# KushalChaudhari-16/Medical-Image-Denoising-Using-Diffusion

Measured on AMD Instinct MI355X. Metric: denoised images/sec, 256x256 x50 DDIM steps, higher is better.
Workload: dtype f32 (split-fp16 x3 MFMA, fp32 accumulate); 1 GPU; batch=8/GPU 256x256 grayscale, 50-iteration reverse loop (noise_steps=50, inference_steps=50), random-init 12.8M-param UNet (BASELINE.json configs[1]); batch_per_gpu=8, global_batch=8, parallelism=single, collective=none

## Files before the change

### medical-image-denoising-using-diffusion_amd/csrc/conv_mfma_f16x3.hip

```cpp
#include "f16x3_common.h"
#include <cstdlib>
#include <type_traits>
#ifdef MIDD_CONV_TIMING
#include <cstdio>
#include <cstring>
#include <string>
#include <vector>
#endif

namespace midd {

template <int KS, int STRIDE, int TW, int MT, int NT, int WM, int WN, int CBT = 0>
struct Conv16Geom {
    static constexpr int NW = WM * WN;
    static constexpr int NTHREADS = NW * 64;
    static constexpr int BM = WM * MT * 16;
    static constexpr int TH = BM / TW;
    static constexpr int IH = (TH - 1) * STRIDE + KS;
    static constexpr int IW = (TW - 1) * STRIDE + KS;
    static constexpr int NPIX = IH * IW;
    static constexpr int CB = CBT ? CBT : conv16_cb(KS);
    static constexpr bool WIDE = (KS == 3 && CB == 2);
    static constexpr int QPP = 4 * CB;
    static constexpr int NSLOT = NPIX * QPP;
// ... 67 lines not shown
    float* const stat_lds = reinterpret_cast<float*>(wring + RING * WSLICE);
    float* const add_lds = stat_lds + G::STAT_FLOATS;
    float* const gnp = add_lds + G::ADD_FLOATS;

    const int tid = threadIdx.x;
    const int lane = tid & 63;
    const int wave = __builtin_amdgcn_readfirstlane(tid >> 6);
    const int wn = wave % WN;
    const int wm = wave / WN;
    const int p16 = lane & 15;
    const int kq = lane >> 4;

    const int tiles_per_img = a.tiles_x * a.tiles_y;
    const int b = blockIdx.x / a.wgs_per_img;
    int trem = blockIdx.x - b * a.wgs_per_img;
    int oy0 = (trem / a.tiles_x) * TH, ox0 = (trem % a.tiles_x) * TW;

    const int Cin = a.C0 + a.C1;
    const int nblk = Cin >> 4;
    constexpr int CB = G::CB, QPP = G::QPP;
    const int nchunks = (nblk + CB - 1) / CB;
    const int ntiles_total = a.Cout >> 4;
    const int ntile_wg = blockIdx.y * (WN * NT);
    const int res_steps = RES ? a.res_steps : 0;
    const int total_steps = conv16_num_steps(Cin, TAPS, G::CB) + res_steps;

    const char* const wbase = reinterpret_cast<const char*>(a.wpack) + (size_t)ntile_wg * 2048;
    const size_t wstep_bytes = (size_t)ntiles_total * 2048;
    const int lane16 = lane * 16;
    int wr_step = 0, wr_slot = 0;
    const char* wr_src = wbase;
#ifdef MIDD_DMA_CHECK
    constexpr unsigned SENT_W = 0x7FFF7FFFu;
    constexpr unsigned SENT_A = 0x7FC0DEADu;
    unsigned dma_bad = 0;
    auto sent4 = [](unsigned v) { typedef unsigned u32x4_ __attribute__((ext_vector_type(4))); return __builtin_bit_cast(f32x4, (u32x4_){v, v, v, v}); };
    auto has_sent = [](const auto& q, unsigned v) {
        typedef unsigned u32x4_ __attribute__((ext_vector_type(4)));
        const u32x4_ u = __builtin_bit_cast(u32x4_, q);
        return (unsigned)((u[0] == v) | (u[1] == v) | (u[2] == v) | (u[3] == v));
    };
#endif
    auto issue_w = [&]() {
        char* slot = wring + wr_slot * WSLICE;
#ifdef MIDD_DMA_CHECK
#pragma unroll
        for (int i = 0; i < PPW; ++i) {
            int piece = (WM == 1) ? wave * PPW + i : wave + i * NW;
            if (piece >= G::WPIECES) piece -= G::WPIECES;
            lds_store_raw(slot + piece * 1024 + lane16, sent4(SENT_W));
        }
// ... 47 lines not shown
            const unsigned byte_off = (unsigned)max(g_off[s], 0) * 64u;
            dma16(base + byte_off, raw + (wave + s * NW) * 1024);
        }
    };
    float rscale = RAW_PRESCALE;
    auto transform = [&](int c) {
        const int blk = CB * c + sblk;
        if (blk >= nblk) return;
        const int ch = (blk << 4) + (q8 & 3) * 4;
        f32x4 rq[APW];
#pragma unroll
        for (int s = 0; s < APW; ++s) rq[s] = *reinterpret_cast<const f32x4*>(raw + (tid + s * NTHREADS) * 16);
#ifdef MIDD_DMA_CHECK
#pragma unroll
        for (int s = 0; s < APW; ++s) dma_bad |= has_sent(rq[s], SENT_A);
#endif
        f32x4 sc = {rscale, rscale, rscale, rscale}, sh = {0.f, 0.f, 0.f, 0.f};
        if (a.prologue != PRO_RAW) {
            sc = *reinterpret_cast<const f32x4*>(gnp + ch);
            sh = *reinterpret_cast<const f32x4*>(gnp + Cin + ch);
        }
        char* base = img + sblk * 2 * PLANE + (q8 & 3) * 8;
        typedef unsigned u32x2 __attribute__((ext_vector_type(2)));
        if (c == 0 && tile_pad) {
#pragma unroll
            for (int s = 0; s < APW; ++s) {
                const int slot = tid + s * NTHREADS;
                if (g_off[s] == -1) {
                    *reinterpret_cast<u32x2*>(base + (slot / QPP) * 32) = (u32x2){0u, 0u};
                    *reinterpret_cast<u32x2*>(base + PLANE + (slot / QPP) * 32) = (u32x2){0u, 0u};
                }
            }
        }
#pragma unroll
        for (int s = 0; s < APW; ++s) {
            const int slot = tid + s * NTHREADS;
            float v[4];
#pragma unroll
            for (int e = 0; e < 4; ++e) v[e] = __builtin_fmaf(rq[s][e], sc[e], sh[e]);
#if defined(C16_ABL) && C16_ABL == 4
            if (false) {
#else
            if (a.prologue == PRO_GN_SILU) {
#endif
#pragma unroll
                for (int e = 0; e < 4; ++e) {
                    const float d = __builtin_fmaf(__builtin_amdgcn_exp2f(v[e]), 1.0f / ACT_PRESCALE, 1.0f / ACT_PRESCALE);
// ... 12 lines not shown
    };

    int frag_base[MT];
#pragma unroll
    for (int mt = 0; mt < MT; ++mt) {
        const int pp = (wm * MT + mt) * 16 + p16;
        const int py = pp / TW, px = pp - py * TW;
        frag_base[mt] = ((py * STRIDE) * IW + px * STRIDE) * 32 + (kq & 1) * 16;
    }
    int frag_full[MT];
#pragma unroll
    for (int mt = 0; mt < MT; ++mt) frag_full[mt] = frag_base[mt] + (kq >> 1) * 2 * PLANE;
    const int wfrag_off = (wn * NT) * 2048 + lane * 16;

    f32x4 acc[MT][NT];
#pragma unroll
    for (int mt = 0; mt < MT; ++mt)
#pragma unroll
        for (int nt = 0; nt < NT; ++nt) acc[mt][nt] = (f32x4){0.f, 0.f, 0.f, 0.f};

    constexpr int D = RING - 1;
    const int ntile0 = ntile_wg + wn * NT;
    TS_DECL
    issue_a(0);
#pragma unroll
    for (int i = 0; i < D; ++i) issue_w();
#if !(defined(C16_ABL) && C16_ABL == 6)
    if (a.prologue == PRO_GN || a.prologue == PRO_GN_SILU)
        gn_prologue_lds(a.gn_tot0, a.C0, a.gn_bs0, a.gn_tot1, a.C1, a.gn_bs1, a.stat_rep, a.gn_gamma, a.gn_beta, a.gn_eps, a.gn_inv_n, b,
                        (a.prologue == PRO_GN_SILU) ? SILU_ARG_FACTOR : ACT_PRESCALE, gnp, tid, NTHREADS, a.status);
#endif
    stat_word* const raw_acc = reinterpret_cast<stat_word*>(gnp);
    if (a.prologue == PRO_RAW && a.gn_tot0 != nullptr && wave == 0)
        raw_sumsq_lds(a.gn_tot0, a.C0, a.gn_bs0, a.gn_tot1, a.C1, a.gn_bs1, a.stat_rep, b, raw_acc, lane);
    stat_word* const res_acc = reinterpret_cast<stat_word*>(gnp + 2 * Cin);
    if (res_steps > 0 && a.res_tot0 != nullptr && wave == NW - 1)
        raw_sumsq_lds(a.res_tot0, a.res_C0, a.res_bs0, a.res_tot1, a.res_C1, a.res_bs1, a.stat_rep, b, res_acc, lane);
    {
        const int trow = (a.temb != nullptr) ? a.trow[b] : 0;
        for (int i = tid; i < G::ADD_FLOATS; i += NTHREADS) {
            const int co = ntile_wg * 16 + i;
            add_lds[i] = a.bias[co] + (a.temb != nullptr ? a.temb[(size_t)trow * a.temb_stride + co] : 0.f);
        }
    }
    wait_vm_and_barrier<0>();
    float oscale = a.out_scale;
    if (a.prologue == PRO_RAW) {
        rscale = a.raw_scale_fixed;
        if (a.gn_tot0 != nullptr) {
            bool bad;
            const int ex = __builtin_amdgcn_readfirstlane(raw_prescale_exp(raw_acc, &bad));
            rscale = pow2f(ex);
            if (bad && tid == 0 && a.status != nullptr) atomicOr(a.status, (int)STATUS_NONFINITE);
        }
        oscale = a.out_scale / rscale;
    }
    float res_in = 1.0f, res_rescale = 1.0f;
    if (res_steps > 0) {
        if (a.res_tot0 != nullptr) {
            bool bad;
            res_in = pow2f(__builtin_amdgcn_readfirstlane(raw_prescale_exp(res_acc, &bad)));
            if (bad && tid == 0 && a.status != nullptr) atomicOr(a.status, (int)STATUS_NONFINITE);
        }
        res_rescale = a.out_scale * res_in / a.res_scale;
        oscale = a.res_scale / res_in;
    }
    transform(0);
    if constexpr (WM == 1) {
        asm volatile("s_waitcnt lgkmcnt(0)" ::: "memory");
        __builtin_amdgcn_s_barrier();
        asm volatile("" ::: "memory");
    }

    TS(TS_PROLOGUE)
    int rd_slot = 0;
    half8 xh[MT], xl[MT];
    auto load_x = [&](const int (&xo)[MT]) {
#pragma unroll
        for (int mt = 0; mt < MT; ++mt) {
            xh[mt] = *reinterpret_cast<const half8*>(img + xo[mt]);
            xl[mt] = *reinterpret_cast<const half8*>(img + xo[mt] + PLANE);
        }
    };
    auto mfma_step = [&]() {
        const char* wslot = wring + rd_slot * WSLICE + wfrag_off;
        rd_slot = (rd_slot + 1 == RING) ? 0 : rd_slot + 1;
        half8 wh[NT], wl[NT];
#pragma unroll
        for (int nt = 0; nt < NT; ++nt) {
            wh[nt] = *reinterpret_cast<const half8*>(wslot + nt * 2048);
// ... 229 lines not shown
                lds_store_raw(my_stat + NT * 16 + nt * 16, ssq[nt]);
            }
        }
        constexpr int ROWF = 2 * NT * 16;
        constexpr int NCOL = WN * NT * 16;
        auto fold = [&](int i) {
            const int which = i / NCOL, col = i - which * NCOL;
            const int wn_i = col / (NT * 16), c = col - wn_i * (NT * 16);
            float t = 0.f;
#pragma unroll
            for (int m = 0; m < WM; ++m) t += stat_lds[(m * WN + wn_i) * ROWF + which * (NT * 16) + c];
            return t;
        };
        static_assert(G::RAW_BYTES + G::IMG_BYTES + RING * WSLICE >= (NCOL + 2) * STAT_WORDS * 8, "block accumulators in the staging buffers (raw, image, ring: contiguous, idle here)");
        if constexpr (G::RAW_BYTES < (NCOL + 2) * STAT_WORDS * 8) {
            asm volatile("s_waitcnt lgkmcnt(0)" ::: "memory");
            __builtin_amdgcn_s_barrier();
            asm volatile("" ::: "memory");
        }
        stat_publish(a.stat_tot, b, a.Cout, a.stat_bs, a.stat_rep, (blockIdx.x - b * a.wgs_per_img) % a.stat_rep, ntile_wg * 16, NCOL,
                     fold, reinterpret_cast<stat_word*>(raw), tid, NTHREADS);
    };

    for (;;) {
        const int next_tile = trem + a.wgs_per_img;
        const bool has_next_tile = next_tile < tiles_per_img;
        for (int c = 0; c < nchunks; ++c) {
            const bool more_in_tile = (c + 1 < nchunks);
            const bool more = more_in_tile || has_next_tile;
            const int next_chunk = more_in_tile ? c + 1 : 0;
            const bool full = (CB == 2) && (2 * c + 1 < nblk);
            if (!more_in_tile && has_next_tile) set_tile(next_tile);
            auto run_chunk = [&](auto more_t) {
                constexpr bool MORE = decltype(more_t)::value;
                if (full) {
#pragma unroll
                    for (int tap = 0; tap < TAPS; ++tap) {
                        const int dy = tap / KS, dx = tap - dy * KS;
                        int xo[MT];
#pragma unroll
                        for (int mt = 0; mt < MT; ++mt) xo[mt] = frag_full[mt] + (dy * IW + dx) * 32;
                        if (MORE && tap >= 1 && tap <= D) k_step(std::true_type{}, false, false, next_chunk, xo);
                        else                              k_step(std::false_type{}, tap == 0, MORE && tap == 0, next_chunk, xo);
                    }
                } else {
#pragma unroll
                    for (int hs = 0; hs < HSTEPS; ++hs) {
                        const int t0 = 2 * hs, t1 = (2 * hs + 1 < TAPS) ? 2 * hs + 1 : 0;
                        const int o0 = ((t0 / KS) * IW + (t0 % KS)) * 32, o1 = ((t1 / KS) * IW + (t1 % KS)) * 32;
                        const int to = (kq >> 1) ? o1 : o0;
                        int xo[MT];
#pragma unroll
                        for (int mt = 0; mt < MT; ++mt) xo[mt] = frag_base[mt] + to;
// ... 18 lines not shown
#ifdef MIDD_CONV_TIMING
                    ts_after_epi = true;
#endif
                }
#if !(defined(C16_ABL) && C16_ABL == 5)
                transform(next_chunk);
#endif
                TS(TS_TRANSFORM)
                if constexpr (WM == 1) {
                    asm volatile("s_waitcnt lgkmcnt(0)" ::: "memory");
                    __builtin_amdgcn_s_barrier();
                    asm volatile("" ::: "memory");
                }
            } else {
                run_chunk(std::false_type{});
                res_phase();
                TS(TS_RES)
            }
        }
        if (!has_next_tile) break;
    }
    asm volatile("s_waitcnt vmcnt(0)" ::: "memory");
    TS(TS_CHUNK_WAIT)
    epilogue();
    TS(TS_EPILOGUE)
    publish_stats();
#ifdef MIDD_DMA_CHECK
    if (dma_bad && a.status != nullptr) atomicOr(a.status, (int)STATUS_DMA_EARLY);
#endif
    TS(TS_PUBLISH)
#ifdef MIDD_CONV_TIMING
    if (tid == 0) {
        ts_acc[TS_TOTAL] = ts_last - ts_t0;
        ts_acc[TS_REAL] = __builtin_amdgcn_s_memrealtime() - ts_r0;
        ts_acc[TS_WGS] = 1;
        for (int k = 0; k < TS_N; ++k) atomicAdd(&g_conv_timing[a.dbg_slot][k], ts_acc[k]);
    }
#endif
}

#ifdef MIDD_CONV_TIMING
static std::vector<std::string> g_timing_names;
static int conv_timing_slot(int ks, int st, int tw, int mt, int nt, int wm, int wn, int oh, int cin, int cout, int B, int ring, int wgs) {
    char buf[160];
    snprintf(buf, sizeof buf, "k%d s%d tile(%d,%d,%d,%d,%d) ring%d out%d^2 %d->%d B%d wgs%d", ks, st, tw, mt, nt, wm, wn, ring, oh, cin, cout, B, wgs);
    for (size_t i = 0; i < g_timing_names.size(); ++i) if (g_timing_names[i] == buf) return (int)i;
    if (g_timing_names.size() >= 63) return 63;
    g_timing_names.push_back(buf);
    return (int)g_timing_names.size() - 1;
// ... 3 lines not shown
    (void)hipDeviceSynchronize();
    (void)hipMemcpyFromSymbol(h, HIP_SYMBOL(g_conv_timing), sizeof h);
    static const char* names[] = {"barrier", "dma-issue", "frag+mfma", "chunk-wait", "transform", "epilogue", "prologue", "wait-after-epi", "dma-wait", "res-phase", "publish"};
    for (size_t i = 0; i < g_timing_names.size(); ++i) {
        const double tot = (double)h[i][TS_TOTAL], wgs = (double)h[i][TS_WGS];
        if (wgs == 0) continue;
        printf("%-70s cyc/wg %9.0f clk %.2f GHz |", g_timing_names[i].c_str(), tot / wgs, tot / (double)h[i][TS_REAL] * 0.1);
        for (int k = 0; k < 11; ++k) printf(" %s %4.1f%%", names[k], 100.0 * (double)h[i][k] / tot);
        printf("\n");
    }
    memset(h, 0, sizeof h);
    (void)hipMemcpyToSymbol(HIP_SYMBOL(g_conv_timing), h, sizeof h);
    fflush(stdout);
}
#endif
template <int KS, int STRIDE, int TW, int MT, int NT, int WM, int WN, bool RES, int CBT = 0>
static hipError_t launch16(const ConvArgs& a0, hipStream_t s) {
    using G = Conv16Geom<KS, STRIDE, TW, MT, NT, WM, WN, CBT>;
    ConvArgs a = a0;
    a.tiles_x = (a.OW + TW - 1) / TW;
    a.tiles_y = (a.OH + G::TH - 1) / G::TH;
    const int ny = a.Cout / (WN * NT * 16);
    a.wgs_per_img = conv16_wgs_per_img(a.tiles_x * a.tiles_y, a.B, ny, a.persist_wgs);
    dim3 grid(a.B * a.wgs_per_img, ny);
#ifdef MIDD_CONV_TIMING
    a.dbg_slot = conv_timing_slot(KS, STRIDE, TW, MT * 10 + G::CB, NT, WM, WN, a.OH, a.C0 + a.C1, a.Cout, a.B, G::RING, (int)grid.x * (int)grid.y);
#endif
    if constexpr (G::LDS_BYTES <= 160 * 1024 && (G::RING - 2) * G::PPW + G::APW <= 60) {
        const int lds_bytes = G::lds_bytes(a.C0 + a.C1);
        if (lds_bytes > 160 * 1024) return hipErrorInvalidValue;
        {
            static int raised[MIDD_MAX_DEVICES] = {};
            hipError_t e = ensure_dynamic_lds(reinterpret_cast<const void*>(&conv_mfma_f16x3_kernel<KS, STRIDE, TW, MT, NT, WM, WN, RES, CBT>), lds_bytes, raised);
            if (e != hipSuccess) return e;
        }
        if ((double)a.H * a.W * 64.0 >= 4294967296.0) return hipErrorInvalidValue;
        hipLaunchKernelGGL((conv_mfma_f16x3_kernel<KS, STRIDE, TW, MT, NT, WM, WN, RES, CBT>), grid, dim3(G::NTHREADS), lds_bytes, s, a);
        return hipGetLastError();
    } else {
        return hipErrorInvalidValue;
    }
}

int conv16_wgs_per_img(int tiles, int B, int ny, int target) {
    const int target_wgs = target ? target : 768;
    int per_img = target_wgs / (B * ny);
    if (per_img < 1) per_img = 1;
// ... 55 lines not shown
        const long wgs = (long)B * tiles * (nn_d / d.wn);
        const long covered = tiles * d.tw * th;
        const bool wasteful = covered * 4 > (long)OH * OW * 5;
        const long share = (long)bm * 8 + d.wn;
        const long score = (wgs >= min_wgs ? 1000000 : wgs * (1000000 / min_wgs)) + share - (wasteful ? 500000 : 0);
        if (score > best_score) { best_score = score; best = &d; best_wgs = wgs; }
    }
    if (!best) return false;
    *t = ConvTile{ks, stride, best->tw, best->mt, best->nt, best->wm, best->wn};
    if (allow_wide && ks == 3 && stride == 1 && best->tw == 16 && best->nt == 3 && best->wm == 4 && best->wn == 1 && Cin >= 32 &&
        best_wgs <= MIDD_WIDE_MAX_WGS && tile16_fits(*best, ks, stride, 2))
        t->cb = 2;
    return true;
}

template <int KS, int STRIDE, int TW, int MT, int NT, int WM, int WN, int CBT = 0>
static bool info16(int Cin, int Cout, int B, int OH, int OW, int persist_wgs, ConvLaunchInfo* o) {
    using G = Conv16Geom<KS, STRIDE, TW, MT, NT, WM, WN, CBT>;
    o->tiles_x = (OW + TW - 1) / TW; o->tiles_y = (OH + G::TH - 1) / G::TH;
    o->grid_y = Cout / (WN * NT * 16);
    o->wgs_per_img = conv16_wgs_per_img(o->tiles_x * o->tiles_y, B, o->grid_y, persist_wgs);
    o->grid_x = B * o->wgs_per_img;
    o->ring = G::RING; o->ppw = G::PPW; o->apw = G::APW; o->lds_bytes = G::lds_bytes(Cin);
    return true;
}
bool conv16_launch_info(int Cin, int Cout, int B, int OH, int OW, const ConvTile& t, int persist_wgs, ConvLaunchInfo* out) {
    if (t.ks == 1 && t.tw == 0) return conv1x1_launch_info(Cin, Cout, B, OH, OW, t, persist_wgs, ATT_NONE, out);
    if (t.cb == 2) {
        if (t.mt == 2) return info16<3, 1, 16, 2, 3, 4, 1, 2>(Cin, Cout, B, OH, OW, persist_wgs, out);
        if (t.mt == 1) return info16<3, 1, 16, 1, 3, 4, 1, 2>(Cin, Cout, B, OH, OW, persist_wgs, out);
        return false;
    }
#define X(tw_, mt_, nt_, wm_, wn_)                                                            \
    if (t.tw == tw_ && t.mt == mt_ && t.nt == nt_ && t.wm == wm_ && t.wn == wn_) {           \
        if (t.ks == 3 && t.stride == 1) return info16<3, 1, tw_, mt_, nt_, wm_, wn_>(Cin, Cout, B, OH, OW, persist_wgs, out); \
        if (t.ks == 3 && t.stride == 2) return info16<3, 2, tw_, mt_, nt_, wm_, wn_>(Cin, Cout, B, OH, OW, persist_wgs, out); \
        if (t.ks == 1 && t.stride == 1) return info16<1, 1, tw_, mt_, nt_, wm_, wn_>(Cin, Cout, B, OH, OW, persist_wgs, out); \
    }
    MIDD_CONV16_TILES(X)
#undef X
    return false;
}

hipError_t conv16_launch(const ConvArgs& a, const ConvTile& t, hipStream_t s) {
    if (t.ks == 1 && t.tw == 0) return conv1x1_launch(a, t, s);
    if (t.cb == 2) {
// ... 19 lines not shown
```

### medical-image-denoising-using-diffusion_amd/csrc/midd_api.hip

```cpp
#include "../../include/midd.h"
#include "midd_internal.h"

#include <cmath>
#include <cstdarg>
#include <cstdio>
#include <cstring>
#include <map>
#include <memory>
#include <mutex>
#include <string>
#include <vector>

using namespace midd;

static const int ATTN_HEADS_ABI = 2;

static thread_local char g_err[512] = "";

static int fail(int code, const char* fmt, ...) {
    va_list ap;
    va_start(ap, fmt);
    vsnprintf(g_err, sizeof(g_err), fmt, ap);
    va_end(ap);
    return code;
// ... 27 lines not shown
};

struct GnRef { size_t gamma = 0, beta = 0; bool on = false; };

enum OpKind { OP_IN_CONV, OP_CONV, OP_ATTN, OP_RESIZE, OP_CONVT, OP_OUT, OP_CHAN_TOT };
struct Op {
    OpKind kind;
    TensorRef s0, s1, dst, resid;
    bool has_s1 = false, has_resid = false;
    GnRef gn;
    size_t partial_off = 0;
    int att_mode = ATT_NONE, att_ksplit = 1, att_tps = 1;
    int stat_rows = 0;
    size_t w = 0, b = 0;
    int prologue = PRO_RAW, temb_col = -1;
    ConvTile tile{};
    int stride = 1, ks = 3;
    bool want_stats = false;
    TensorRef res0, res1;
    bool has_res1 = false; int res_steps = 0; float res_scale = 1.f;
    bool raw_stats = false;
    float raw_scale_fixed = 1.f;
    float out_scale = 1.f;
};

constexpr int INVARIANT_B = 4;

struct Program {
    int B, H, W;
    int persist_wgs = 0;
    bool wide_chunks = false;
    std::vector<Op> ops;
    size_t bytes = 0, trow_off = 0;
    size_t stats_off = 0, stats_bytes = 0;
    int stat_rep = 1;
    std::map<std::string, TensorRef> outputs;
};

struct mi_plan {
    mi_unet_cfg cfg{};
    bool batch_invariant = false;
    std::vector<Mod> downs, mid, ups;
    int final_c = 0, temb_cols = 0, levels = 0;
    std::vector<std::string> expected;
    std::map<std::string, std::vector<int64_t>> expected_shape;
    std::map<std::string, HostWeight> host;
    float* wdev = nullptr; size_t wdev_floats = 0;
    float* ttab = nullptr; int time_rows = 0;
    size_t w_in = 0, b_in = 0, g_out = 0, be_out = 0, w_out = 0, b_out = 0;
    bool finalized = false;
    int device = -1;
    std::mutex mu;
    std::map<uint64_t, std::unique_ptr<Program>> programs;
    static const int MAX_PARTS = 4;
// ... 498 lines not shown
    int conv(const TensorRef& s0, const TensorRef* s1, TensorRef& dst, size_t w, size_t b, float wscale, int ks, int stride,
             int prologue, GnRef gn, int temb_col, const TensorRef* resid, bool want_stats, float raw_scale_fixed = 1.0f,
             int att_mode = ATT_NONE, size_t att_scratch = 0, int att_ksplit = 1) {
        Op o{}; o.kind = OP_CONV; o.att_mode = att_mode; o.partial_off = att_scratch; o.att_ksplit = att_ksplit; o.s0 = s0; if (s1) { o.s1 = *s1; o.has_s1 = true; }
        o.out_scale = (prologue == PRO_RAW && p->cfg.compute_mode == MI_COMPUTE_F16X3) ? wscale * ACT_PRESCALE_H : wscale;
        o.raw_scale_fixed = raw_scale_fixed;
        o.raw_stats = prologue == PRO_RAW && s0.stat_id >= 0 && (!s1 || s1->stat_id >= 0);
        o.w = w; o.b = b; o.ks = ks; o.stride = stride; o.prologue = prologue; o.temb_col = temb_col; o.gn = gn;
        if (gn.on) { if (int rcg = gn_consumer(s0, s1)) return rcg; }
        if (resid) { o.resid = *resid; o.has_resid = true; }
        const int Bp = p->batch_invariant ? INVARIANT_B : B;
        const size_t w_wide = next_wide; next_wide = (size_t)-1;
        const bool ok = (p->cfg.compute_mode == MI_COMPUTE_F16X3)
                            ? conv16_pick_tile(s0.C + (s1 ? s1->C : 0), dst.C, Bp, dst.H, dst.W, ks, stride, &o.tile, g->wide_chunks && w_wide != (size_t)-1)
                            : conv_pick_tile(dst.C, Bp, dst.H, dst.W, ks, stride, &o.tile);
        if (!ok) return fail(MI_EINVAL, "no conv tile for Cout=%d ks=%d stride=%d", dst.C, ks, stride);
        if (o.tile.cb == 2) o.w = w_wide;
        if (att_mode == ATT_PART_IN) o.tile.mt = 1;
        if (want_stats) { alloc_stats(dst); o.want_stats = true; }
        o.dst = dst;
        g->ops.push_back(o);
        return MI_OK;
    }
};

static int build_program(mi_plan* p, int B, int H, int W, Program* g) {
    const mi_unet_cfg& c = p->cfg;
    const int div = 1 << (p->levels - 1);
    if (B < 1 || H < div || W < div || H % div || W % div)
        return fail(MI_EINVAL, "H and W must be positive multiples of %d (got %dx%d), B >= 1", div, H, W);
    g->B = B; g->H = H; g->W = W;
    g->stat_rep = (640 / B + 47) / 48;
    if (g->stat_rep < 1) g->stat_rep = 1;
    if (g->stat_rep > STAT_MAX_REPLICAS) g->stat_rep = STAT_MAX_REPLICAS;
    Builder bld{p, g, Bump{}, B};
    (void)bld.bump.take(256);
    g->trow_off = bld.bump.take((size_t)B * sizeof(int));
    int rc;

    const GnRef no_gn{};
    auto run_rb = [&](const Mod& m, const TensorRef& s0, const TensorRef* s1, TensorRef* out) -> int {
        const int cin = s0.C + (s1 ? s1->C : 0);
        if (cin != m.in_c) return fail(MI_EINVAL, "%s: expected %d input channels, graph provides %d", m.name.c_str(), m.in_c, cin);
        TensorRef h1 = bld.alloc(m.out_c, s0.H, s0.W);
        TensorRef o = bld.alloc(m.out_c, s0.H, s0.W);
        const GnRef g2{m.g2, m.be2, true};
// ... 91 lines not shown
                bld.next_wide = pending_up->wcx;
                if ((rc = bld.conv(h, nullptr, o, pending_up->wc, pending_up->bc, pending_up->sc, 3, 1, PRO_RAW, no_gn, -1, nullptr, true))) return rc;
                h = o; pending_up = nullptr;
            } else if ((rc = flush_up())) return rc;
        }
        if (h.H != skip.H || h.W != skip.W) {
            TensorRef o = bld.alloc(h.C, skip.H, skip.W);
            bld.alloc_stats(o);
            Op op{}; op.kind = OP_RESIZE; op.s0 = h; op.dst = o; g->ops.push_back(op);
            h = o;
        }
        TensorRef o; if ((rc = run_rb(m, h, &skip, &o))) return rc;
        h = o; g->outputs[m.name] = h;
    }
    if ((rc = flush_up())) return rc;
    if (h.H != H || h.W != W) return fail(MI_EINVAL, "network output is %dx%d for a %dx%d input", h.H, h.W, H, W);
    if ((rc = bld.gn_consumer(h, nullptr))) return rc;
    { Op o{}; o.kind = OP_OUT; o.s0 = h; o.gn = GnRef{p->g_out, p->be_out, true}; g->ops.push_back(o); }
    size_t cur = 0;
    for (auto& st : bld.stats) {
        st.off = cur;
        cur += ((size_t)B * (st.C / st.bs) * g->stat_rep * STAT_WORDS * sizeof(stat_word) + 255) & ~(size_t)255;
    }
    g->stats_bytes = cur;
    g->stats_off = bld.bump.take(g->stats_bytes);
    auto resolve = [&](TensorRef& t) {
        if (t.stat_id >= 0) { t.tot_off = g->stats_off + bld.stats[t.stat_id].off; t.stat_bs = bld.stats[t.stat_id].bs; }
    };
    for (Op& o : g->ops) for (TensorRef* t : {&o.s0, &o.s1, &o.dst, &o.resid, &o.res0, &o.res1}) resolve(*t);
    for (auto& kv : g->outputs) resolve(kv.second);
    g->bytes = (bld.bump.cur + 255) & ~(size_t)255;
    return MI_OK;
}

static int get_program(mi_plan* p, int B, int H, int W, Program** out, bool side_by_side = false) {
    if (!p->finalized) return fail(MI_ESTATE, "mi_unet_finalize has not been called (or weights changed since)");
    static const bool plan_as_side = getenv("MIDD_PLAN_AS_SIDE") != nullptr;
    side_by_side = side_by_side || plan_as_side;
    const uint64_t key = ((uint64_t)(side_by_side ? 1 : 0) << 63) ^ ((uint64_t)B << 40) ^ ((uint64_t)H << 20) ^ (uint64_t)W;
    std::lock_guard<std::mutex> lk(p->mu);
    auto it = p->programs.find(key);
    if (it == p->programs.end()) {
        std::unique_ptr<Program> g(new Program());
        g->persist_wgs = side_by_side ? 640 : 0;
        if (p->batch_invariant) g->persist_wgs = 640 / INVARIANT_B * B;
        g->wide_chunks = !side_by_side && !p->batch_invariant;
        int rc = build_program(p, B, H, W, g.get());
        if (rc) return rc;
        it = p->programs.emplace(key, std::move(g)).first;
    }
    *out = it->second.get();
    return MI_OK;
}

static int split_parts(int B) {
    static const int want = getenv("MIDD_SPLIT") ? atoi(getenv("MIDD_SPLIT")) : 2;
    int parts = (want >= 4) ? 4 : (want >= 2 ? 2 : 1);
    while (parts > 1 && (B % parts || B / parts < 2)) parts /= 2;
    return parts;
}

extern "C" size_t mi_workspace_bytes(mi_plan* plan, int B, int H, int W) {
    Program* g = nullptr;
    if (!plan || get_program(plan, B, H, W, &g)) return 0;
    size_t need = g->bytes;
    const int parts = split_parts(B);
    if (parts > 1) {
        Program* gh = nullptr;
        if (get_program(plan, B / parts, H, W, &gh, true)) return 0;
// ... 41 lines not shown
        case OP_ATTN: {
            const double N = (double)o.dst.H * o.dst.W;
            snprintf(buf, sizeof(buf), "midd::attention_%s_kernel<%d>", p->cfg.compute_mode == MI_COMPUTE_F16X3 ? "f16x3" : "f32", o.dst.C / 2);
            *name = buf;
            *flops = 4.0 * B * N * N * o.dst.C;
            *bytes = 4.0 * (elems(o.s0) + elems(o.dst));
            break;
        }
        case OP_RESIZE: *name = "midd::resize_bilinear_kernel"; *flops = 0; *bytes = 4.0 * (elems(o.s0) + elems(o.dst)); break;
        case OP_CONVT:
            *name = "midd::conv_transpose_kernel";
            *flops = 2.0 * elems(o.s0) * o.dst.C * 16; *bytes = 4.0 * (elems(o.s0) + elems(o.dst));
            break;
        case OP_OUT:
            *name = p->cfg.in_channels == 1 ? "midd::out_conv_kernel<1>" : "midd::out_conv_kernel<0>";
            *flops = 2.0 * B * g->H * g->W * o.s0.C * 9 * p->cfg.in_channels;
            *bytes = 4.0 * (elems(o.s0) + 3.0 * B * p->cfg.in_channels * g->H * g->W);
            break;
    }
}

static int dump_program(mi_plan* p, int B, int H, int W, bool side_by_side, std::string* out) {
    Program g;
    g.persist_wgs = side_by_side ? 640 : 0;
    if (p->batch_invariant) g.persist_wgs = 640 / INVARIANT_B * B;
    g.wide_chunks = !side_by_side && !p->batch_invariant;
    int rc = build_program(p, B, H, W, &g);
    if (rc) return rc;
    char line[512];
    snprintf(line, sizeof line, "program B=%d %dx%d side=%d bytes=%zu stats_off=%zu stats_bytes=%zu stat_rep=%d persist_wgs=%d wide=%d ops=%zu\n",
             B, H, W, (int)side_by_side, g.bytes, g.stats_off, g.stats_bytes, g.stat_rep, g.persist_wgs, (int)g.wide_chunks, g.ops.size());
    *out += line;
    static const char* kinds[] = {"in_conv", "conv", "attn", "resize", "convT", "out", "chan_tot"};
    int idx = 0;
    for (const Op& o : g.ops) {
        std::string name; double fl, by;
        op_work(p, &g, o, &name, &fl, &by);
        int n = snprintf(line, sizeof line, "op%03d %-8s %dx%d c%d+%d->%d k%d s%d pro%d res_steps%d att%d ksplit%d tps%d bs(in %d,%d out %d) | %s",
                         idx++, kinds[o.kind], o.dst.H ? o.dst.H : H, o.dst.W ? o.dst.W : W, o.s0.C, o.has_s1 ? o.s1.C : 0, o.dst.C, o.ks, o.stride,
                         o.prologue, o.res_steps, o.att_mode, o.att_ksplit, o.att_tps, o.s0.stat_bs, o.has_s1 ? o.s1.stat_bs : 0, o.dst.stat_bs, name.c_str());
        if (o.kind == OP_CONV && p->cfg.compute_mode == MI_COMPUTE_F16X3) {
            ConvLaunchInfo li{};
            if (conv16_launch_info(o.s0.C + (o.has_s1 ? o.s1.C : 0), o.dst.C, B, o.dst.H, o.dst.W, o.tile, g.persist_wgs, &li))
                n += snprintf(line + n, sizeof line - n, " | grid %dx%d wgs/img %d tiles %dx%d ring %d ppw %d apw %d lds %d", li.grid_x, li.grid_y, li.wgs_per_img,
                              li.tiles_x, li.tiles_y, li.ring, li.ppw, li.apw, li.lds_bytes);
        }
        snprintf(line + n, sizeof line - n, "\n");
        *out += line;
    }
    return MI_OK;
}
extern "C" int mi_debug_conv16_geometry(int ks, int stride, int tw, int mt, int nt, int wm, int wn, int cb, int* ring, int* ppw, int* apw, int* lds_bytes) {
    if (!ring || !ppw || !apw || !lds_bytes) return fail(MI_EINVAL, "null argument");
    ConvTile t{ks, stride, tw, mt, nt, wm, wn, cb};
    ConvLaunchInfo li{};
    if (!conv16_launch_info(384, 16 * nt * wn, 1, 64, 64, t, 0, &li)) return fail(MI_EINVAL, "tile (%d,%d,%d,%d,%d) ks %d stride %d cb %d is not instantiated", tw, mt, nt, wm, wn, ks, stride, cb);
    *ring = li.ring; *ppw = li.ppw; *apw = li.apw; *lds_bytes = li.lds_bytes;
    return MI_OK;
}
extern "C" int mi_debug_plan_dump(mi_plan* plan, int B, int H, int W, int side_by_side, char* buf, size_t cap) {
    if (!plan) return fail(MI_EINVAL, "null plan");
    std::string text;
    int rc = dump_program(plan, B, H, W, side_by_side != 0, &text);
    if (rc) return rc;
    if (buf && cap) { snprintf(buf, cap, "%s", text.c_str()); }
    return (int)text.size();
}

static int run_program(mi_plan* p, Program* g, const StepIO& io, char* ws, int* status, hipStream_t s,
                       hipEvent_t mid_event = nullptr, int mid_div = 2) {
// ... 42 lines not shown
                        a.res_tot1 = o.has_res1 ? T(o.res1.tot_off) : T(o.res0.tot_off); a.res_bs1 = o.has_res1 ? o.res1.stat_bs : 1;
                    }
                }
                if (o.att_mode != ATT_NONE) {
                    const Att16Layout lay = attention16_layout(B, o.dst.H * o.dst.W, o.att_mode == ATT_QKV_OUT ? o.dst.C / 3 : o.dst.C);
                    a.att_mode = o.att_mode; a.att_heads = ATTN_HEADS_ABI; a.att_D = (o.att_mode == ATT_QKV_OUT ? o.dst.C / 3 : o.dst.C) / ATTN_HEADS_ABI;
                    a.att_npad = lay.npad; a.att_ksplit = o.att_ksplit;
                    a.att_k = reinterpret_cast<_Float16*>(ws + o.partial_off + lay.k_off); a.att_v = reinterpret_cast<_Float16*>(ws + o.partial_off + lay.v_off);
                    a.att_ml = reinterpret_cast<const float*>(ws + o.partial_off + lay.ml_off);
                }
                if (o.gn.on || o.raw_stats) {
                    a.gn_tot0 = T(o.s0.tot_off); a.gn_bs0 = o.s0.stat_bs;
                    a.gn_tot1 = o.has_s1 ? T(o.s1.tot_off) : T(o.s0.tot_off); a.gn_bs1 = o.has_s1 ? o.s1.stat_bs : 1;
                }
                if (o.gn.on) {
                    a.gn_gamma = wd + o.gn.gamma; a.gn_beta = wd + o.gn.beta; a.gn_eps = 1e-5f;
                    a.gn_inv_n = 1.0 / ((double)o.s0.H * o.s0.W * ((a.C0 + a.C1) / GN_GROUPS_));
                }
                if (o.temb_col >= 0) { a.temb = p->ttab + o.temb_col; a.temb_stride = p->temb_cols; a.trow = reinterpret_cast<const int*>(ws + g->trow_off); }
                a.resid = o.has_resid ? F(o.resid.off) : nullptr;
                a.out = F(o.dst.off); a.out_scale = o.out_scale;
                if (o.want_stats) { a.stat_tot = T(o.dst.tot_off); a.stat_bs = o.dst.stat_bs; }
                a.persist_wgs = g->persist_wgs;
                e = (p->cfg.compute_mode == MI_COMPUTE_F16X3) ? conv16_launch(a, o.tile, s) : conv_launch(a, o.tile, s);
                break;
            }
            case OP_ATTN:
                if (p->cfg.compute_mode == MI_COMPUTE_F16X3) {
                    const int N = o.dst.H * o.dst.W, C = o.dst.C;
                    const Att16Layout lay = attention16_layout(B, N, C);
                    char* sc = ws + o.partial_off;
                    e = attention16_launch(F(o.s0.off), reinterpret_cast<const _Float16*>(sc + lay.k_off), reinterpret_cast<const _Float16*>(sc + lay.v_off),
                                           reinterpret_cast<float*>(sc + lay.po_off), reinterpret_cast<float*>(sc + lay.ml_off),
                                           B, o.att_ksplit, o.att_tps, N, C, ATTN_HEADS_ABI, s);
                } else {
                    e = attention_launch(F(o.s0.off), F(o.dst.off), B, o.dst.H * o.dst.W, o.dst.C, 2, s);
                }
                break;
            case OP_RESIZE:
                e = resize_bilinear_launch(F(o.s0.off), F(o.dst.off), T(o.dst.tot_off), g->stat_rep, o.dst.stat_bs, B, o.s0.H, o.s0.W, o.s0.C, o.dst.H, o.dst.W, blocked, s);
                break;
            case OP_CONVT:
                e = conv_transpose_launch(F(o.s0.off), wd + o.w, wd + o.b, F(o.dst.off), B, o.s0.H, o.s0.W, o.s0.C, o.dst.C, blocked, s);
                break;
            case OP_OUT: {
                OutConvArgs a{};
// ... 227 lines not shown
```

### medical-image-denoising-using-diffusion_amd/csrc/midd_internal.h

```cpp
#pragma once
#include <hip/hip_runtime.h>
#include <stdint.h>
#include "stats_common.h"

namespace midd {

constexpr int MIDD_MAX_DEVICES = 64;
inline hipError_t ensure_dynamic_lds(const void* kernel, int bytes, int (&raised)[MIDD_MAX_DEVICES]) {
    if (bytes <= 64 * 1024) return hipSuccess;
    int dev = 0;
    hipError_t e = hipGetDevice(&dev);
    if (e != hipSuccess) return e;
    if (dev < 0 || dev >= MIDD_MAX_DEVICES) return hipErrorInvalidDevice;
    if (bytes > raised[dev]) {
        e = hipFuncSetAttribute(kernel, hipFuncAttributeMaxDynamicSharedMemorySize, bytes);
        if (e != hipSuccess) return e;
        raised[dev] = bytes;
    }
    return hipSuccess;
}

enum Prologue { PRO_RAW = 0, PRO_GN = 1, PRO_GN_SILU = 2 };

__host__ __device__ inline size_t act_index(int blocked, int b, int C, int HW, int pix, int ch) {
    return blocked ? (((size_t)b * (C >> 4) + (ch >> 4)) * HW + pix) * 16 + (ch & 15) : ((size_t)b * HW + pix) * C + ch;
}

struct ConvArgs {
    const float* src0;
    const float* src1;
    int C0, C1;
    int B, H, W;
    int OH, OW;
    const float* wpack;
    const float* bias;
    int Cout;
    const stat_word* gn_tot0; const stat_word* gn_tot1;
    int gn_bs0, gn_bs1;
    float raw_scale_fixed;
    int* status;
    const float* gn_gamma; const float* gn_beta; float gn_eps; double gn_inv_n;
    int prologue;
    const float* temb;
    int temb_stride;
    const int* trow;
    const float* resid;
    float* out;
    float out_scale;
    stat_word* stat_tot;
    int stat_rep;
    int stat_bs;
    const float* res_src0; const float* res_src1;
    int res_C0, res_C1, res_steps;
    float res_scale;
    const stat_word* res_tot0; const stat_word* res_tot1;
    int res_bs0, res_bs1;
    int att_mode;
    _Float16* att_k; _Float16* att_v;
    const float* att_ml;
    int att_heads, att_D, att_npad, att_ksplit;
    int tiles_x, tiles_y;
    int wgs_per_img;
    int persist_wgs;
#ifdef MIDD_CONV_TIMING
    int dbg_slot;
#endif
};

struct ConvTile {
    int ks, stride, tw, mt, nt, wm, wn;
    int cb = 0;
};

enum ComputeMode { MODE_F32 = 0, MODE_F16X3 = 1 };
enum AttMode { ATT_NONE = 0, ATT_QKV_OUT = 1, ATT_PART_IN = 2 };
enum StatusBits { STATUS_NONFINITE = 1, STATUS_FP16_RANGE = 2,
                  STATUS_DMA_EARLY = 4 };

bool conv_pick_tile(int Cout, int B, int OH, int OW, int ks, int stride, ConvTile* t);
hipError_t conv_launch(const ConvArgs& a, const ConvTile& t, hipStream_t s);

bool conv16_pick_tile(int Cin, int Cout, int B, int OH, int OW, int ks, int stride, ConvTile* t, bool allow_wide = false);
int conv16_wgs_per_img(int tiles, int B, int ny, int target = 0);
bool conv1x1_pick_tile(int Cin, int Cout, int B, int OH, int OW, ConvTile* t);
hipError_t conv1x1_launch(const ConvArgs& a, const ConvTile& t, hipStream_t s);
hipError_t conv16_launch(const ConvArgs& a, const ConvTile& t, hipStream_t s);
struct ConvLaunchInfo { int grid_x, grid_y, wgs_per_img, tiles_x, tiles_y, ring, ppw, apw, lds_bytes; };
bool conv16_launch_info(int Cin, int Cout, int B, int OH, int OW, const ConvTile& t, int persist_wgs, ConvLaunchInfo* out);
bool conv1x1_launch_info(int Cin, int Cout, int B, int OH, int OW, const ConvTile& t, int persist_wgs, int att_mode, ConvLaunchInfo* out);
__host__ __device__ constexpr int conv16_cb(int ks) { return ks == 1 ? 2 : 1; }
__host__ __device__ inline int conv16_num_steps(int Cin, int taps, int cb = 0) {
    const int nblk = Cin / 16;
    if (cb == 0) cb = conv16_cb(taps == 1 ? 1 : 3);
    if (cb == 1) return nblk * ((taps + 1) / 2);
    const int full = nblk / 2, half = nblk & 1;
    return full * taps + half * ((taps + 1) / 2);
}

constexpr int GN_GROUPS_ = 8;
hipError_t chan_total_launch(const float* src, stat_word* tot, int rep, int bs, int B, int HW, int C, int rows, int blocked, hipStream_t s);
int chan_partial_rows(int HW, int C);

size_t resize_workspace_bytes(int n, int sw, int sh, int dw, int dh);
hipError_t resize_bicubic_u8_launch(const unsigned char* src, int n, int sw, int sh, unsigned char* dst, int dw, int dh, void* ws, hipStream_t s);
hipError_t u8_to_unit_launch(const unsigned char* src, float* dst, size_t count, hipStream_t s);
hipError_t unit_to_u8_launch(const float* src, unsigned char* dst, size_t count, hipStream_t s);
size_t metrics_workspace_bytes(int n, int h);
hipError_t metrics_launch(const float* target, const float* pred, int n, int h, int w, double* out, void* ws, hipStream_t s);

hipError_t attention_launch(const float* qkv, float* out, int B, int N, int C, int heads, hipStream_t s);
// ... 33 lines not shown
```

Before: 49.90 images/s.

## Add split-K partitioning over input-channel chunks for 3x3 f16x3 convolutions

Adds a third grid dimension so 3x3 stride-1 convolutions can split their input-channel chunks across up to four workgroups. Each part writes partial accumulators to a global slab and takes an atomic ticket; the last part to arrive sums all partials and runs the epilogue and stats publishing. The host picks the number of parts per op automatically from tile count against a workgroup target, aiming to fill the GPU on small-resolution layers. The cost is extra global traffic for the partials, atomics and a serial reduction in the last workgroup, plus reliance on the ticket counters being reset between launches.

Result: slower. 45.33 images/s, median of 2 (-9.2%).

```diff
diff --git a/medical-image-denoising-using-diffusion_amd/csrc/conv_mfma_f16x3.hip b/medical-image-denoising-using-diffusion_amd/csrc/conv_mfma_f16x3.hip
--- a/medical-image-denoising-using-diffusion_amd/csrc/conv_mfma_f16x3.hip
+++ b/medical-image-denoising-using-diffusion_amd/csrc/conv_mfma_f16x3.hip
@@ -113,11 +113,17 @@
     const int nchunks = (nblk + CB - 1) / CB;
     const int ntiles_total = a.Cout >> 4;
     const int ntile_wg = blockIdx.y * (WN * NT);
-    const int res_steps = RES ? a.res_steps : 0;
-    const int total_steps = conv16_num_steps(Cin, TAPS, G::CB) + res_steps;
-
-    const char* const wbase = reinterpret_cast<const char*>(a.wpack) + (size_t)ntile_wg * 2048;
+    const int kparts = a.kparts > 1 ? a.kparts : 1;
+    const int part = kparts > 1 ? (int)blockIdx.z : 0;
+    const int c_lo = kparts > 1 ? a.kchunk[part] : 0;
+    const int c_hi = kparts > 1 ? a.kchunk[part + 1] : nchunks;
+    constexpr int CHUNK_STEPS = (CB == 2) ? TAPS : HSTEPS;
+    const int launch_res = RES ? a.res_steps : 0;
+    const int res_steps = (part == kparts - 1) ? launch_res : 0;
+    const int total_steps = (c_hi == nchunks ? conv16_num_steps(Cin, TAPS, G::CB) : c_hi * CHUNK_STEPS) - c_lo * CHUNK_STEPS + res_steps;
+
     const size_t wstep_bytes = (size_t)ntiles_total * 2048;
+    const char* const wbase = reinterpret_cast<const char*>(a.wpack) + (size_t)ntile_wg * 2048 + (size_t)(c_lo * CHUNK_STEPS) * wstep_bytes;
     const int lane16 = lane * 16;
     int wr_step = 0, wr_slot = 0;
     const char* wr_src = wbase;
@@ -211,7 +217,7 @@
         }
         char* base = img + sblk * 2 * PLANE + (q8 & 3) * 8;
         typedef unsigned u32x2 __attribute__((ext_vector_type(2)));
-        if (c == 0 && tile_pad) {
+        if (c == c_lo && tile_pad) {
 #pragma unroll
             for (int s = 0; s < APW; ++s) {
                 const int slot = tid + s * NTHREADS;
@@ -270,7 +276,7 @@
     constexpr int D = RING - 1;
     const int ntile0 = ntile_wg + wn * NT;
     TS_DECL
-    issue_a(0);
+    issue_a(c_lo);
 #pragma unroll
     for (int i = 0; i < D; ++i) issue_w();
 #if !(defined(C16_ABL) && C16_ABL == 6)
@@ -282,7 +288,7 @@
     if (a.prologue == PRO_RAW && a.gn_tot0 != nullptr && wave == 0)
         raw_sumsq_lds(a.gn_tot0, a.C0, a.gn_bs0, a.gn_tot1, a.C1, a.gn_bs1, a.stat_rep, b, raw_acc, lane);
     stat_word* const res_acc = reinterpret_cast<stat_word*>(gnp + 2 * Cin);
-    if (res_steps > 0 && a.res_tot0 != nullptr && wave == NW - 1)
+    if (launch_res > 0 && a.res_tot0 != nullptr && wave == NW - 1)
         raw_sumsq_lds(a.res_tot0, a.res_C0, a.res_bs0, a.res_tot1, a.res_C1, a.res_bs1, a.stat_rep, b, res_acc, lane);
     {
         const int trow = (a.temb != nullptr) ? a.trow[b] : 0;
@@ -304,7 +310,7 @@
         oscale = a.out_scale / rscale;
     }
     float res_in = 1.0f, res_rescale = 1.0f;
-    if (res_steps > 0) {
+    if (launch_res > 0) {
         if (a.res_tot0 != nullptr) {
             bool bad;
             res_in = pow2f(__builtin_amdgcn_readfirstlane(raw_prescale_exp(res_acc, &bad)));
@@ -313,7 +319,7 @@
         res_rescale = a.out_scale * res_in / a.res_scale;
         oscale = a.res_scale / res_in;
     }
-    transform(0);
+    transform(c_lo);
     if constexpr (WM == 1) {
         asm volatile("s_waitcnt lgkmcnt(0)" ::: "memory");
         __builtin_amdgcn_s_barrier();
@@ -589,13 +595,65 @@
                      fold, reinterpret_cast<stat_word*>(raw), tid, NTHREADS);
     };
 
+    auto split_finish = [&]() -> bool {
+        const int items = gridDim.x * gridDim.y;
+        const int item = blockIdx.x + gridDim.x * blockIdx.y;
+        constexpr int ITEM_BYTES = NW * MT * NT * 1024;
+        const int tile_off = wave * (MT * NT * 1024) + lane16;
+        char* const slab = reinterpret_cast<char*>(a.kslab);
+        if (launch_res > 0 && res_steps == 0) {
+#pragma unroll
+            for (int mt = 0; mt < MT; ++mt)
+#pragma unroll
+                for (int nt = 0; nt < NT; ++nt) acc[mt][nt] *= res_rescale;
+        }
+        {
+            typedef unsigned u32x4 __attribute__((ext_vector_type(4)));
+            const __amdgpu_buffer_rsrc_t rs = __builtin_amdgcn_make_buffer_rsrc(slab + ((size_t)part * items + item) * ITEM_BYTES, (short)0, ITEM_BYTES, 0x00020000);
+#pragma unroll
+            for (int mt = 0; mt < MT; ++mt)
+#pragma unroll
+                for (int nt = 0; nt < NT; ++nt)
+                    __builtin_amdgcn_raw_buffer_store_b128(__builtin_bit_cast(u32x4, acc[mt][nt]), rs, tile_off + (mt * NT + nt) * 1024, 0, 16 );
+        }
+        int* const kflag = reinterpret_cast<int*>(gnp + 2 * Cin);
+        asm volatile("s_waitcnt vmcnt(0)" ::: "memory");
+        __builtin_amdgcn_s_barrier();
+        asm volatile("" ::: "memory");
+        if (tid == 0) {
+            const int ticket = atomicAdd(a.kticket + item, 1);
+            if (ticket == kparts - 1) __builtin_amdgcn_fence(__ATOMIC_ACQUIRE, "agent");
+            *kflag = ticket;
+        }
+        asm volatile("s_waitcnt vmcnt(0) lgkmcnt(0)" ::: "memory");
+        __builtin_amdgcn_s_barrier();
+        asm volatile("" ::: "memory");
+        if (__builtin_amdgcn_readfirstlane(*kflag) != kparts - 1) return false;
+        f32x4 sum[MT][NT];
+        for (int p = 0; p < kparts; ++p) {
+            const char* src = slab + ((size_t)p * items + item) * ITEM_BYTES + tile_off;
+#pragma unroll
+            for (int mt = 0; mt < MT; ++mt)
+#pragma unroll
+                for (int nt = 0; nt < NT; ++nt) {
+                    const f32x4 v = (p == part) ? acc[mt][nt] : *reinterpret_cast<const f32x4*>(src + (mt * NT + nt) * 1024);
+                    sum[mt][nt] = (p == 0) ? v : sum[mt][nt] + v;
+                }
+        }
+#pragma unroll
+        for (int mt = 0; mt < MT; ++mt)
+#pragma unroll
+            for (int nt = 0; nt < NT; ++nt) acc[mt][nt] = sum[mt][nt];
+        return true;
+    };
+
     for (;;) {
         const int next_tile = trem + a.wgs_per_img;
         const bool has_next_tile = next_tile < tiles_per_img;
-        for (int c = 0; c < nchunks; ++c) {
-            const bool more_in_tile = (c + 1 < nchunks);
+        for (int c = c_lo; c < c_hi; ++c) {
+            const bool more_in_tile = (c + 1 < c_hi);
             const bool more = more_in_tile || has_next_tile;
-            const int next_chunk = more_in_tile ? c + 1 : 0;
+            const int next_chunk = more_in_tile ? c + 1 : c_lo;
             const bool full = (CB == 2) && (2 * c + 1 < nblk);
             if (!more_in_tile && has_next_tile) set_tile(next_tile);
             auto run_chunk = [&](auto more_t) {
@@ -660,9 +718,11 @@
     }
     asm volatile("s_waitcnt vmcnt(0)" ::: "memory");
     TS(TS_CHUNK_WAIT)
-    epilogue();
-    TS(TS_EPILOGUE)
-    publish_stats();
+    if (kparts == 1 || split_finish()) {
+        epilogue();
+        TS(TS_EPILOGUE)
+        publish_stats();
+    }
 #ifdef MIDD_DMA_CHECK
     if (dma_bad && a.status != nullptr) atomicOr(a.status, (int)STATUS_DMA_EARLY);
 #endif
@@ -712,7 +772,10 @@
     a.tiles_y = (a.OH + G::TH - 1) / G::TH;
     const int ny = a.Cout / (WN * NT * 16);
     a.wgs_per_img = conv16_wgs_per_img(a.tiles_x * a.tiles_y, a.B, ny, a.persist_wgs);
-    dim3 grid(a.B * a.wgs_per_img, ny);
+    const int kparts = a.kparts > 1 ? a.kparts : 1;
+    if (kparts > 1 && (kparts > KPARTS_MAX || STRIDE != 1 || a.wgs_per_img != a.tiles_x * a.tiles_y || !a.kslab || !a.kticket))
+        return hipErrorInvalidValue;
+    dim3 grid(a.B * a.wgs_per_img, ny, kparts);
 #ifdef MIDD_CONV_TIMING
     a.dbg_slot = conv_timing_slot(KS, STRIDE, TW, MT * 10 + G::CB, NT, WM, WN, a.OH, a.C0 + a.C1, a.Cout, a.B, G::RING, (int)grid.x * (int)grid.y);
 #endif
@@ -814,6 +877,31 @@
     o->wgs_per_img = conv16_wgs_per_img(o->tiles_x * o->tiles_y, B, o->grid_y, persist_wgs);
     o->grid_x = B * o->wgs_per_img;
     o->ring = G::RING; o->ppw = G::PPW; o->apw = G::APW; o->lds_bytes = G::lds_bytes(Cin);
+    o->nw = G::NW; o->mt = MT; o->nt = NT;
+    return true;
+}
+
+bool conv16_kchunks(int Cin, int cb, int res_steps, int kparts, int min_steps, int* kchunk) {
+    if (kparts < 1 || kparts > KPARTS_MAX) return false;
+    const int nblk = Cin / 16;
+    if (cb == 0) cb = conv16_cb(3);
+    const int nchunks = (nblk + cb - 1) / cb;
+    const int cs = cb == 2 ? 9 : 5;
+    const int steps = conv16_num_steps(Cin, 9, cb);
+    if (nchunks < kparts) return false;
+    const double per_part = (double)(steps + res_steps) / kparts;
+    int last = kparts == 1 ? nchunks : (int)((per_part - res_steps) / cs + 0.5);
+    if (last < 1) last = 1;
+    if (last > nchunks - (kparts - 1)) last = nchunks - (kparts - 1);
+    const int rest = nchunks - last, each = kparts > 1 ? rest / (kparts - 1) : 0, extra = kparts > 1 ? rest % (kparts - 1) : 0;
+    kchunk[0] = 0;
+    for (int p = 0; p < kparts - 1; ++p) kchunk[p + 1] = kchunk[p] + each + (p < extra ? 1 : 0);
+    kchunk[kparts] = nchunks;
+    for (int p = 0; p < kparts; ++p) {
+        const int c_lo = kchunk[p], c_hi = kchunk[p + 1];
+        const int st = (c_hi == nchunks ? steps : c_hi * cs) - c_lo * cs + (p == kparts - 1 ? res_steps : 0);
+        if (c_hi <= c_lo || st < min_steps) return false;
+    }
     return true;
 }
 bool conv16_launch_info(int Cin, int Cout, int B, int OH, int OW, const ConvTile& t, int persist_wgs, ConvLaunchInfo* out) {
diff --git a/medical-image-denoising-using-diffusion_amd/csrc/midd_api.hip b/medical-image-denoising-using-diffusion_amd/csrc/midd_api.hip
--- a/medical-image-denoising-using-diffusion_amd/csrc/midd_api.hip
+++ b/medical-image-denoising-using-diffusion_amd/csrc/midd_api.hip
@@ -73,6 +73,8 @@
     bool raw_stats = false;
     float raw_scale_fixed = 1.f;
     float out_scale = 1.f;
+    int kparts = 1, kchunk[KPARTS_MAX + 1] = {};
+    size_t kticket_off = 0, kslab_bytes = 0;
 };
 
 constexpr int INVARIANT_B = 4;
@@ -81,6 +83,8 @@
     int B, H, W;
     int persist_wgs = 0;
     bool wide_chunks = false;
+    int kparts_cap_pct = 100;
+    size_t kslab_off = 0, kslab_bytes = 0;
     std::vector<Op> ops;
     size_t bytes = 0, trow_off = 0;
     size_t stats_off = 0, stats_bytes = 0;
@@ -625,6 +629,28 @@
         g->ops.push_back(o);
         return MI_OK;
     }
+    void choose_kparts(Op& o) {
+        o.kparts = 1;
+        if (p->cfg.compute_mode != MI_COMPUTE_F16X3 || o.kind != OP_CONV || o.ks != 3 || o.stride != 1 || o.tile.tw == 0) return;
+        static const int knob = getenv("MIDD_KPARTS") ? atoi(getenv("MIDD_KPARTS")) : 0;
+        if (knob == 1) return;
+        const int cin = o.s0.C + (o.has_s1 ? o.s1.C : 0);
+        ConvLaunchInfo li{};
+        if (!conv16_launch_info(cin, o.dst.C, B, o.dst.H, o.dst.W, o.tile, g->persist_wgs, &li)) return;
+        if (li.wgs_per_img != li.tiles_x * li.tiles_y) return;
+        const double per_sample_target = (double)(g->persist_wgs ? g->persist_wgs : 768) / B;
+        const double cap = per_sample_target * g->kparts_cap_pct / 100.0;
+        const int per_sample = li.wgs_per_img * li.grid_y;
+        for (int k = KPARTS_MAX; k >= 2; --k) {
+            if (knob >= 2 ? k != (knob > KPARTS_MAX ? KPARTS_MAX : knob) : per_sample * k > cap) continue;
+            int kc[KPARTS_MAX + 1];
+            if (!conv16_kchunks(cin, o.tile.cb, o.res_steps, k, li.ring, kc)) continue;
+            o.kparts = k;
+            for (int i = 0; i <= k; ++i) o.kchunk[i] = kc[i];
+            o.kslab_bytes = (size_t)k * li.grid_x * li.grid_y * li.nw * li.mt * li.nt * 1024;
+            return;
+        }
+    }
 };
 
 static int build_program(mi_plan* p, int B, int H, int W, Program* g) {
@@ -762,8 +788,18 @@
         st.off = cur;
         cur += ((size_t)B * (st.C / st.bs) * g->stat_rep * STAT_WORDS * sizeof(stat_word) + 255) & ~(size_t)255;
     }
+    for (Op& o : g->ops) {
+        bld.choose_kparts(o);
+        if (o.kparts <= 1) continue;
+        const size_t items = o.kslab_bytes / ((size_t)o.kparts * 1024);
+        o.kticket_off = cur;
+        cur += (items * sizeof(int) + 255) & ~(size_t)255;
+        if (o.kslab_bytes > g->kslab_bytes) g->kslab_bytes = o.kslab_bytes;
+    }
     g->stats_bytes = cur;
     g->stats_off = bld.bump.take(g->stats_bytes);
+    for (Op& o : g->ops) if (o.kparts > 1) o.kticket_off += g->stats_off;
+    if (g->kslab_bytes) g->kslab_off = bld.bump.take(g->kslab_bytes);
     auto resolve = [&](TensorRef& t) {
         if (t.stat_id >= 0) { t.tot_off = g->stats_off + bld.stats[t.stat_id].off; t.stat_bs = bld.stats[t.stat_id].bs; }
     };
@@ -771,6 +807,16 @@
     for (auto& kv : g->outputs) resolve(kv.second);
     g->bytes = (bld.bump.cur + 255) & ~(size_t)255;
     return MI_OK;
+}
+
+#ifndef MIDD_KPARTS_CAP_PCT
+#define MIDD_KPARTS_CAP_PCT 150
+#endif
+static void setup_program(const mi_plan* p, Program* g, int B, bool side_by_side) {
+    g->persist_wgs = side_by_side ? 640 : 0;
+    if (p->batch_invariant) g->persist_wgs = 640 / INVARIANT_B * B;
+    g->wide_chunks = !side_by_side && !p->batch_invariant;
+    g->kparts_cap_pct = g->persist_wgs ? MIDD_KPARTS_CAP_PCT : 100;
 }
 
 static int get_program(mi_plan* p, int B, int H, int W, Program** out, bool side_by_side = false) {
@@ -782,9 +828,7 @@
     auto it = p->programs.find(key);
     if (it == p->programs.end()) {
         std::unique_ptr<Program> g(new Program());
-        g->persist_wgs = side_by_side ? 640 : 0;
-        if (p->batch_invariant) g->persist_wgs = 640 / INVARIANT_B * B;
-        g->wide_chunks = !side_by_side && !p->batch_invariant;
+        setup_program(p, g.get(), B, side_by_side);
         int rc = build_program(p, B, H, W, g.get());
         if (rc) return rc;
         it = p->programs.emplace(key, std::move(g)).first;
@@ -872,9 +916,7 @@
 
 static int dump_program(mi_plan* p, int B, int H, int W, bool side_by_side, std::string* out) {
     Program g;
-    g.persist_wgs = side_by_side ? 640 : 0;
-    if (p->batch_invariant) g.persist_wgs = 640 / INVARIANT_B * B;
-    g.wide_chunks = !side_by_side && !p->batch_invariant;
+    setup_program(p, &g, B, side_by_side);
     int rc = build_program(p, B, H, W, &g);
     if (rc) return rc;
     char line[512];
@@ -886,16 +928,25 @@
     for (const Op& o : g.ops) {
         std::string name; double fl, by;
         op_work(p, &g, o, &name, &fl, &by);
-        int n = snprintf(line, sizeof line, "op%03d %-8s %dx%d c%d+%d->%d k%d s%d pro%d res_steps%d att%d ksplit%d tps%d bs(in %d,%d out %d) | %s",
+        char kp[48] = "kparts1";
+        if (o.kparts > 1) {
+            int m = snprintf(kp, sizeof kp, "kparts%d kc", o.kparts);
+            for (int i = 0; i <= o.kparts && m < (int)sizeof kp; ++i) m += snprintf(kp + m, sizeof kp - m, i ? "/%d" : "%d", o.kchunk[i]);
+        }
+        const int cap = (int)sizeof line;
+        int n = snprintf(line, sizeof line, "op%03d %-8s %dx%d c%d+%d->%d k%d s%d pro%d res_steps%d att%d ksplit%d tps%d bs(in %d,%d out %d) %s | %s",
                          idx++, kinds[o.kind], o.dst.H ? o.dst.H : H, o.dst.W ? o.dst.W : W, o.s0.C, o.has_s1 ? o.s1.C : 0, o.dst.C, o.ks, o.stride,
-                         o.prologue, o.res_steps, o.att_mode, o.att_ksplit, o.att_tps, o.s0.stat_bs, o.has_s1 ? o.s1.stat_bs : 0, o.dst.stat_bs, name.c_str());
+                         o.prologue, o.res_steps, o.att_mode, o.att_ksplit, o.att_tps, o.s0.stat_bs, o.has_s1 ? o.s1.stat_bs : 0, o.dst.stat_bs, kp, name.c_str());
+        if (n < 0 || n >= cap) n = cap - 1;
         if (o.kind == OP_CONV && p->cfg.compute_mode == MI_COMPUTE_F16X3) {
             ConvLaunchInfo li{};
-            if (conv16_launch_info(o.s0.C + (o.has_s1 ? o.s1.C : 0), o.dst.C, B, o.dst.H, o.dst.W, o.tile, g.persist_wgs, &li))
-                n += snprintf(line + n, sizeof line - n, " | grid %dx%d wgs/img %d tiles %dx%d ring %d ppw %d apw %d lds %d", li.grid_x, li.grid_y, li.wgs_per_img,
-                              li.tiles_x, li.tiles_y, li.ring, li.ppw, li.apw, li.lds_bytes);
-        }
-        snprintf(line + n, sizeof line - n, "\n");
+            if (conv16_launch_info(o.s0.C + (o.has_s1 ? o.s1.C : 0), o.dst.C, B, o.dst.H, o.dst.W, o.tile, g.persist_wgs, &li)) {
+                const int m = snprintf(line + n, cap - n, " | grid %dx%d wgs/img %d tiles %dx%d ring %d ppw %d apw %d lds %d", li.grid_x, li.grid_y, li.wgs_per_img,
+                                       li.tiles_x, li.tiles_y, li.ring, li.ppw, li.apw, li.lds_bytes);
+                n = (m < 0 || n + m >= cap) ? cap - 1 : n + m;
+            }
+        }
+        snprintf(line + n, cap - n, "\n");
         *out += line;
     }
     return MI_OK;
@@ -984,6 +1035,11 @@
                 a.out = F(o.dst.off); a.out_scale = o.out_scale;
                 if (o.want_stats) { a.stat_tot = T(o.dst.tot_off); a.stat_bs = o.dst.stat_bs; }
                 a.persist_wgs = g->persist_wgs;
+                if (o.kparts > 1) {
+                    a.kparts = o.kparts;
+                    for (int i = 0; i <= o.kparts; ++i) a.kchunk[i] = o.kchunk[i];
+                    a.kslab = F(g->kslab_off); a.kticket = reinterpret_cast<int*>(ws + o.kticket_off);
+                }
                 e = (p->cfg.compute_mode == MI_COMPUTE_F16X3) ? conv16_launch(a, o.tile, s) : conv_launch(a, o.tile, s);
                 break;
             }
diff --git a/medical-image-denoising-using-diffusion_amd/csrc/midd_internal.h b/medical-image-denoising-using-diffusion_amd/csrc/midd_internal.h
--- a/medical-image-denoising-using-diffusion_amd/csrc/midd_internal.h
+++ b/medical-image-denoising-using-diffusion_amd/csrc/midd_internal.h
@@ -25,6 +25,8 @@
 __host__ __device__ inline size_t act_index(int blocked, int b, int C, int HW, int pix, int ch) {
     return blocked ? (((size_t)b * (C >> 4) + (ch >> 4)) * HW + pix) * 16 + (ch & 15) : ((size_t)b * HW + pix) * C + ch;
 }
+
+constexpr int KPARTS_MAX = 4;
 
 struct ConvArgs {
     const float* src0;
@@ -62,6 +64,10 @@
     int tiles_x, tiles_y;
     int wgs_per_img;
     int persist_wgs;
+    int kparts;
+    int kchunk[KPARTS_MAX + 1];
+    float* kslab;
+    int* kticket;
 #ifdef MIDD_CONV_TIMING
     int dbg_slot;
 #endif
@@ -85,7 +91,8 @@
 bool conv1x1_pick_tile(int Cin, int Cout, int B, int OH, int OW, ConvTile* t);
 hipError_t conv1x1_launch(const ConvArgs& a, const ConvTile& t, hipStream_t s);
 hipError_t conv16_launch(const ConvArgs& a, const ConvTile& t, hipStream_t s);
-struct ConvLaunchInfo { int grid_x, grid_y, wgs_per_img, tiles_x, tiles_y, ring, ppw, apw, lds_bytes; };
+struct ConvLaunchInfo { int grid_x, grid_y, wgs_per_img, tiles_x, tiles_y, ring, ppw, apw, lds_bytes, nw, mt, nt; };
+bool conv16_kchunks(int Cin, int cb, int res_steps, int kparts, int min_steps, int* kchunk);
 bool conv16_launch_info(int Cin, int Cout, int B, int OH, int OW, const ConvTile& t, int persist_wgs, ConvLaunchInfo* out);
 bool conv1x1_launch_info(int Cin, int Cout, int B, int OH, int OW, const ConvTile& t, int persist_wgs, int att_mode, ConvLaunchInfo* out);
 __host__ __device__ constexpr int conv16_cb(int ks) { return ks == 1 ? 2 : 1; }
```
